# NILOIDE/A.I.gar

Measured on AMD Instinct MI355X. Metric: env-steps/sec at 4096 bots x 100k pellets; 1/2/4/8 MI355X scaling, higher is better.
Workload: dtype f64; 1 GPU; C3: 4096 bots, 100000 pellets, 1152 viruses, split p=0.0025, eject p=0.01, field 4800, obs 854 floats/bot; start: data/c3_t50.npz (tick 50, mean cell mass 17.45, max 51.3) + 30 untimed random-policy ticks to settle; policy=random, parallelism=single-gpu

## Files before the change

aigar_amd/csrc/aigar_dev.h:

```cpp
#pragma once
#include <stdint.h>

#include "../../include/aigar.h"

namespace aigar {

#ifdef AIGAR_FLOOR
#ifdef AIGAR_FLOOR_OPAQUE
#define FLOOR(k) \
  if ((((AIGAR_FLOOR) >> (k)) & 1) && d.A > 0) return
#else
#define FLOOR(k) \
  if (((AIGAR_FLOOR) >> (k)) & 1) return
#endif
#else
#define FLOOR(k)
#endif

struct ArenaCtl {
  int64_t seq_next;
  int64_t tick;
  int64_t tick_sp;
  uint64_t key0, key1, ctr_pellet, ctr_virus;
  int64_t seq_base_upd;
// ... 91 lines not shown
  int tile_flags;
  int tile_nx, tile_ny;
  int tile_gate;
  int hcap, hrec, nh;
  int *t_holder;
  int *t_obsby;
  int *t_holive;
  uint8_t *t_hodefer;
  int *t_hoslot;
  int own_bx0, own_bx1, own_by0, own_by1;
  int loc_bx0, loc_bx1, loc_by0, loc_by1;
  TileRec *outbox;
  const TileRec *inbox;
  int *ticket;
  int *kill_list;
  double *spec_x, *spec_y, *spec_m;
  double pow_n032[17];
  int cshift;
  int cshift_c;
  int Pcap, Ecap, Vcap, Wcap, EVcap;
  int PR;
  int PS;
  int PD;
  int PH1;
  int virus_enabled;
  double max_pellets, max_viruses;
  int G, L;
  uint32_t obs_ch, obs_ex;
  int flags;
  int pp_par;
  ArenaCtl *ctl;
  int *p_alive, *p_respawn, *p_ncells, *p_split, *p_eject, *p_pend;
  double *p_cmdx, *p_cmdy;
  double *p_fx, *p_fy, *p_fs, *p_mass;
  int *p_split_lh;
  uint8_t *p_role;
  int *p_time;
  double *o_last_mass;
  uint8_t *p_list;
  int *p_newc, *p_newb, *p_seqoff, *p_bloboff;
  int *p_heavy;
  double *c_x, *c_y, *c_m, *c_r, *c_vx, *c_vy, *c_svx, *c_svy, *c_mt;
  int *c_svc;
  uint32_t *c_flags;
  int64_t *c_seq;
  uint8_t *c_active;
  double *sp_r, *sp_svx, *sp_svy;
  double *sb_x, *sb_y, *sb_svx, *sb_svy;
  uint8_t *sb_slot;
  PelRec *pel;
  int *pel_col;
  PelRec *pn;
  int *pn_col;
  uint8_t *pel_dead;
  int *pel_rank;
  int *pstart;
  int *pncnt;
  uint64_t *pel_owner;
  double *b_x, *b_y, *b_m, *b_r, *b_vx, *b_vy, *b_svx, *b_svy;
  int *b_svc;
  int64_t *b_seq, *b_ej;
  int *b_col;
  uint32_t *b_flags;
  uint64_t *b_owner;
  int *bstart, *bitems, *b_rank;
  uint64_t *bmap;
  double *v_x, *v_y, *v_m, *v_r, *v_vx, *v_vy, *v_svx, *v_svy;
  int *v_svc;
  int64_t *v_seq;
  uint32_t *v_flags;
  int *v_active;
  int *vcnt, *vstart, *vitems, *v_rank;
  int *ccnt, *cstart, *citems, *c_rank;
  int *cgcnt;
  unsigned long long *occ;
  int *occ_cnt;
  int occ_words;
  int *dead;
  int *work, *work2;
  int *f_list;
  uint8_t *f_cnt;
  uint8_t *f_done;
  int *resp_slot;
  int64_t *ev;
  double *o_lastfov;
  double *o_self_lf, *o_self_slf, *o_en_lf, *o_en_slf;
  double *o_act_cur, *o_act_prev;
  unsigned long long *scan_state;
  unsigned long long *pl_state;
  int pl_tiles;
  int scan_tiles;
  int OBcap;
  unsigned long long *ob_used;
  uint32_t *ob_epoch;
  int64_t *ob_seq;
  double *ob_m, *ob_r;
  uint32_t *ob_mask;
  uint8_t *ob_own;
  int *ob_perm;
  uint64_t *ob_wmask;
  double *sc;
  ScoreCtl *sc_ctl;
};
enum { SC_N = 0, SC_SUM = 1, SC_MAX = 2, SC_DEAD = 3 };

constexpr int FCAP = 32;

struct RandomPolicy {
  int on;
  double ps, pe;
  uint64_t salt;
};

}
```

aigar_amd/csrc/api.hip:

```cpp
#include <dlfcn.h>
#include <hip/hip_runtime.h>

#include <algorithm>
#include <cmath>
#include <cstdarg>
#include <cstdio>
#include <cstdlib>
#include <cstring>
#include <string>
#include <type_traits>
#include <vector>

#include "../../include/aigar.h"
#include "aigar_dev.h"
#include "aigar_sem.h"

namespace aigar {
void launch_tick(const Dev &d, hipStream_t s, int rounds, int64_t *scr_k, int *scr_v,
                 const RandomPolicy *rp = nullptr);
void launch_tick_pre(const Dev &d, hipStream_t s, int64_t *scr_k, int *scr_v, const RandomPolicy *rp);
void launch_tick_post(const Dev &d, hipStream_t s, int64_t *scr_k, int *scr_v);
void launch_tile_pass(const Dev &d, hipStream_t s, int rounds, int64_t *scr_k, int *scr_v, int first);
void launch_tile_policy(const Dev &d, hipStream_t s, int greedy_split, uint8_t *mask, int cap);
void launch_tile_cmd_apply(const Dev &d, hipStream_t s, int box_recs);
// ... 441 lines not shown
    d.own_bx1 = (ix + 1) * d.cols / tx;
    d.own_by0 = iy * d.cols / ty;
    d.own_by1 = (iy + 1) * d.cols / ty;
    d.loc_bx0 = std::max(0, d.own_bx0 - hb);
    d.loc_bx1 = std::min(d.cols, d.own_bx1 + hb);
    d.loc_by0 = std::max(0, d.own_by0 - hb);
    d.loc_by1 = std::min(d.cols, d.own_by1 + hb);
  }
  d.tile_nx = tx;
  d.tile_ny = ty;
  d.tile_gate = 0;
  d.tcap = cfg->tile_cap > 0 ? cfg->tile_cap : 2048;
  d.bm_words = (int)(((size_t)kMaxCells * d.NP + 255) / 256 * 4);
  {
    const uint32_t ch = cfg->obs_channels;
    d.nh = ((ch & (AIGAR_OBS_SELF_LF | AIGAR_OBS_SELF_SLF)) ? 1 : 0) + ((ch & AIGAR_OBS_SELF_SLF) ? 1 : 0) +
           ((ch & (AIGAR_OBS_ENEMY_LF | AIGAR_OBS_ENEMY_SLF)) ? 1 : 0) + ((ch & AIGAR_OBS_ENEMY_SLF) ? 1 : 0);
    d.hrec = 1 + (d.nh * G * G + 3) / 4;
    d.hcap = std::min(kHcapMax, std::max(16, d.tcap / 64));
  }
  h->box_recs = 1 + d.tcap + std::max(d.bm_words / 4, d.hcap * d.hrec);
  for (int k = 0; k <= kMaxCells; k++) d.pow_n032[k] = aigar_math::pow_glibc((double)k, 0.32);
  d.cshift = 3;
  while ((((d.cols + (1 << d.cshift) - 1) >> d.cshift) * ((d.cols + (1 << d.cshift) - 1) >> d.cshift)) > 4096)
    d.cshift++;
  d.cshift_c = 0;
  while ((((d.cols + (1 << d.cshift_c) - 1) >> d.cshift_c) * ((d.cols + (1 << d.cshift_c) - 1) >> d.cshift_c)) > 4096)
    d.cshift_c++;
  if (hipStreamCreateWithFlags(&h->stream, hipStreamNonBlocking) != hipSuccess) {
    delete h;
    return fail("hipStreamCreate failed");
  }
  const size_t A = d.A, NP = d.NP, C = (size_t)kMaxCells * NP, H1 = (size_t)d.H + 1, GG = (size_t)G * G;
  bool ok = true;
#define AL(field, T, n)                     \
  do {                                      \
    d.field = dalloc<T>(h, (n));            \
    ok = ok && d.field != nullptr;          \
  } while (0)
#ifndef AIGAR_NO_ARENA
  for (int pass = 0; pass < 2; pass++) {
    h->arena_sizing = pass == 0;
    if (pass == 1) {
      h->arena_size = h->arena_used;
      h->arena_used = 0;
      void *base = nullptr;
      if (hipMalloc(&base, h->arena_size) != hipSuccess) {
        ok = false;
        break;
      }
      h->allocs.push_back(base);
      (void)hipMemset(base, 0, h->arena_size);
      h->arena = (char *)base;
    }
#endif
  AL(ctl, ArenaCtl, A);
  AL(p_alive, int, NP); AL(p_respawn, int, NP); AL(p_ncells, int, NP); AL(p_split, int, NP); AL(p_eject, int, NP);
  AL(p_pend, int, NP); AL(p_cmdx, double, NP); AL(p_cmdy, double, NP); AL(p_list, uint8_t, C);
  AL(p_newc, int, NP); AL(p_heavy, int, NP); AL(p_newb, int, NP); AL(p_seqoff, int, NP); AL(p_bloboff, int, NP);
  AL(c_x, double, C); AL(c_y, double, C); AL(c_m, double, C); AL(c_r, double, C); AL(c_vx, double, C);
  AL(c_vy, double, C); AL(c_svx, double, C); AL(c_svy, double, C); AL(c_mt, double, C); AL(c_svc, int, C);
  AL(c_flags, uint32_t, C); AL(c_seq, int64_t, C); AL(c_active, uint8_t, C);
  AL(sp_r, double, C); AL(sp_svx, double, C); AL(sp_svy, double, C);
  AL(sb_x, double, C); AL(sb_y, double, C); AL(sb_svx, double, C); AL(sb_svy, double, C); AL(sb_slot, uint8_t, C);
  const size_t P = A * d.Pcap, PSA = A * d.PS, PDA = A * d.PD, PHA = A * d.PH1;
  AL(pel, PelRec, PSA); AL(pel_col, int, PSA);
  AL(pn, PelRec, P); AL(pn_col, int, P);
  AL(pel_dead, uint8_t, PDA); AL(pel_rank, int, P); AL(pncnt, int, PHA); AL(pstart, int, PHA);
  AL(pel_owner, uint64_t, PDA);
  const size_t E = A * d.Ecap, V = A * d.Vcap;
  AL(b_x, double, E); AL(b_y, double, E); AL(b_m, double, E); AL(b_r, double, E); AL(b_vx, double, E);
  AL(b_vy, double, E); AL(b_svx, double, E); AL(b_svy, double, E); AL(b_svc, int, E); AL(b_seq, int64_t, E);
  AL(b_ej, int64_t, E); AL(b_flags, uint32_t, E); AL(b_owner, uint64_t, E); AL(b_col, int, E);
  AL(bstart, int, A * H1); AL(bitems, int, E); AL(b_rank, int, E); AL(bmap, uint64_t, A * 64);
  AL(v_x, double, V); AL(v_y, double, V); AL(v_m, double, V); AL(v_r, double, V); AL(v_vx, double, V);
  AL(v_vy, double, V); AL(v_svx, double, V); AL(v_svy, double, V); AL(v_svc, int, V); AL(v_seq, int64_t, V);
  AL(v_flags, uint32_t, V); AL(v_active, int, V);
  AL(vcnt, int, A * H1); AL(vstart, int, A * H1); AL(vitems, int, V); AL(v_rank, int, V);
  AL(ccnt, int, A * H1); AL(cstart, int, A * H1); AL(citems, int, C); AL(c_rank, int, C);
  AL(cgcnt, int, A * 2 * 4100);
  AL(occ, unsigned long long, A * d.occ_words); AL(occ_cnt, int, A * d.H);
  AL(dead, int, NP); AL(work, int, A * d.Wcap); AL(work2, int, A * d.Wcap);
  AL(f_list, int, C * FCAP); AL(f_cnt, uint8_t, C); AL(f_done, uint8_t, C);
  AL(resp_slot, int, NP);
  AL(ev, int64_t, A * d.EVcap * 5);
  AL(o_lastfov, double, NP); AL(o_self_lf, double, NP * GG); AL(o_self_slf, double, NP * GG);
  AL(o_en_lf, double, NP * GG); AL(o_en_slf, double, NP * GG); AL(o_act_cur, double, NP * 4);
  AL(o_act_prev, double, NP * 4);
  d.OBcap = (int)std::min<size_t>(std::max<size_t>(1u << 20, 64 * NP), (size_t)1 << 24);
  AL(scan_state, unsigned long long, 2 * A * d.scan_tiles);
  AL(pl_state, unsigned long long, A * d.pl_tiles);
  AL(ticket, int, 16);
  AL(kill_list, int, P); AL(spec_x, double, A * 64); AL(spec_y, double, A * 64); AL(spec_m, double, A * 64); 
  AL(ob_used, unsigned long long, 1);
  AL(ob_epoch, uint32_t, 1);
  AL(p_split_lh, int, NP);
  AL(p_role, uint8_t, NP);
  AL(p_time, int, NP);
  AL(o_last_mass, double, NP);
  if (d.tiled) {
    AL(t_holder, int, NP);
    AL(t_obsby, int, NP);
    AL(t_holive, int, NP);
    AL(t_hodefer, uint8_t, NP);
    AL(t_hoslot, int, d.hcap);
    AL(outbox, TileRec, h->box_recs);
    TileRec *ib = nullptr;
    ib = dalloc<TileRec>(h, (size_t)h->box_recs * d.ntiles);
    ok = ok && ib != nullptr;
    d.inbox = ib;
  }
  AL(p_fx, double, NP); AL(p_fy, double, NP); AL(p_fs, double, NP); AL(p_mass, double, NP); AL(ob_seq, int64_t, d.OBcap); AL(ob_m, double, d.OBcap); AL(ob_r, double, d.OBcap);
  AL(ob_mask, uint32_t, d.OBcap); AL(ob_own, uint8_t, d.OBcap); AL(ob_perm, int, d.OBcap);
  d.ob_wmask = nullptr;
  if (G > 16) AL(ob_wmask, uint64_t, 4 * (size_t)d.OBcap);
  d.sc = nullptr;
  d.sc_ctl = nullptr;
  if (cfg->flags & AIGAR_FLAG_SCORE) {
    AL(sc, double, 4 * NP);
    AL(sc_ctl, ScoreCtl, 1);
  }
#undef AL
  h->scr_k = dalloc<int64_t>(h, A * d.Wcap);
  h->scr_v = dalloc<int>(h, A * d.Wcap);
  h->d_cmd = dalloc<double>(h, NP * 4);
  h->d_mask = dalloc<uint8_t>(h, NP);
  h->d_nnmask = dalloc<uint8_t>(h, NP);
  h->d_stats = dalloc<double>(h, NP * 5);
  h->d_obs = dalloc<double>(h, NP * (size_t)d.L);
  h->d_rlist = dalloc<int>(h, A);
  h->d_rseed = dalloc<uint64_t>(h, A);
  if (d.sc) {
    h->d_score = dalloc<double>(h, NP * 4);
    ok = ok && h->d_score;
  }
  ok = ok && h->scr_k && h->scr_v && h->d_cmd && h->d_stats && h->d_obs && h->d_mask && h->d_nnmask && h->d_rlist &&
       h->d_rseed;
#ifndef AIGAR_NO_ARENA
  }
  h->arena_sizing = false;
  h->arena = nullptr;
#endif
  if (ok) (void)hipMemset(h->d_nnmask, 1, NP);
  if (ok && !d.tiled) {
    ok = hipHostMalloc((void **)&h->h_reset, aigar_handle::kResetSlots * A * 2 * sizeof(uint64_t),
                       hipHostMallocDefault) == hipSuccess;
    for (hipEvent_t &e : h->ev_reset) ok = ok && hipEventCreateWithFlags(&e, hipEventDisableTiming) == hipSuccess;
  }
  (void)hipEventCreate(&h->ev0);
  (void)hipEventCreate(&h->ev1);
  if (!ok) {
    free_all(h);
    delete h;
    return fail("aigar_create: device allocation failed");
  }
  if (hipDeviceSynchronize() != hipSuccess) {
    free_all(h);
    delete h;
    return fail("aigar_create: device synchronize failed");
  }
  *out = h;
  return 0;
}

extern "C" int aigar_destroy(aigar_handle *h) {
  if (!h) return 0;
  (void)hipSetDevice(h->cfg.device);
// ... 3367 lines not shown
```

aigar_amd/csrc/tick.hip:

```cpp
#include <hip/hip_runtime.h>

#include "aigar_dev.h"
#include "aigar_sem.h"
#include "aigar_wave.h"

namespace aigar {

#define GTID ((int)(blockIdx.x * blockDim.x + threadIdx.x))
#define TILE_GATE(d)                                          \
  do {                                                        \
    if ((d).tile_gate && (d).ctl[0].n_undone_glob == 0) return; \
  } while (0)

#ifdef AIGAR_PHASE_TIMING
constexpr int kPtWaves = 8192;
__device__ unsigned int g_ptw[9][kPtWaves][8];
__device__ unsigned int g_ptid[9][kPtWaves][2];
__device__ __forceinline__ void pt_ids(unsigned *o) {
  unsigned a, b;
  asm volatile("s_getreg_b32 %0, hwreg(HW_REG_HW_ID)" : "=s"(a));
  asm volatile("s_getreg_b32 %0, hwreg(HW_REG_XCC_ID)" : "=s"(b));
  o[0] = a;
  o[1] = b;
}
// ... 3717 lines not shown
        }
        nt += __popcll(bal);
      }
      if (nt > PPT_CAP) {
        if (lane == 0) set_err(d, a, ERR_CAND_CAP);
        nt = PPT_CAP;
      }
      tab.n = nt;
      wave_fence();
      pp_group_turns(d, a, mine, g_key[w], g_val[w], g_srt[w], odirty, rmax, d.dead + (size_t)a * d.B + dead0,
                     scr_k + (size_t)a * d.Wcap, &s_nd, tab);
    }
    if (lane == 0) s_rmax[w] = rmax;
  }
  __syncthreads();
  PT_SUB(5);
  PT_MARK(5, 7);
  const int nd = s_nd;
  const int64_t *dk = scr_k + (size_t)a * d.Wcap;
  int *dl = d.dead + (size_t)a * d.B + dead0;
  int rk[2], pv[2];
  for (int k = 0; k < 2; k++) {
    const int i = tid + k * T;
    rk[k] = -1;
    if (i < nd) {
      const int64_t key = dk[i];
      int r = 0;
      for (int j = 0; j < nd; j++) r += dk[j] < key;
      rk[k] = r;
      pv[k] = dl[i];
    }
  }
  if (nd > 2 * T && tid == 0) set_err(d, a, ERR_WORK_CAP);
  __syncthreads();
  for (int k = 0; k < 2; k++)
    if (rk[k] >= 0) dl[rk[k]] = pv[k];
  if (tid == 0) {
    double r = c.rmax_cell;
    for (int k = 0; k < PPG_WAVES; k++) r = fmax(r, s_rmax[k]);
    c.rmax_cell = r;
    c.n_dead = dead0 + nd;
    c.stat[6] += 1;
  }
  PT_SUB(6);
}

__device__ void spawn_pos(const Dev &d, int a, double radius, const uint64_t u[4], double &ox, double &oy) {
  const int cols = d.cols, total = d.H;
  const unsigned long long *occ = d.occ + (size_t)a * d.occ_words;
  int sb = (int)mulhi(u[0], (uint64_t)total);
  int found = -1;
  for (int pass = 0; pass < 2 && found < 0; pass++) {
    int lo = pass == 0 ? sb : 0, hi = pass == 0 ? total : sb;
    for (int b = lo; b < hi && found < 0;) {
      int wd = b >> 6;
      unsigned long long free_bits = ~occ[wd];
      free_bits &= (~0ull) << (b & 63);
      int wend = (wd + 1) << 6;
      if (wend > hi) free_bits &= (hi - (wd << 6)) >= 64 ? ~0ull : ((1ull << (hi - (wd << 6))) - 1);
      if (free_bits) found = (wd << 6) + __ffsll((long long)free_bits) - 1;
      b = wend;
    }
  }
  int64_t xp, yp;
  if (found < 0) {
    xp = ph_randint(u[1], 0, d.size);
    yp = ph_randint(u[2], 0, d.size);
  } else {
    int64_t x = found % cols;
    double y = (double)(found - x) / cols;
    int64_t left = (x - 1) * kBucket;
    double top = y * kBucket;
    xp = ph_randint(u[1], left + radius, (double)(left + kBucket) - radius);
    yp = ph_randint(u[2], top + radius, top + kBucket - radius);
  }
  ox = (double)xp;
  oy = (double)yp;
}

struct SpawnIn {
  int n_pel, n_pel_eaten, n_pnew, n_pel_glob, n_eaten_glob, n_vir;
  int64_t seq_next, tick, stat3, stat5;
  uint64_t ctr_pellet, ctr_virus;
  int n_spawn_p;
};
__device__ __forceinline__ SpawnIn spawn_in(const ArenaCtl &c) {
  return SpawnIn{c.n_pel,    c.n_pel_eaten, c.n_pnew,    c.n_pel_glob, c.n_eaten_glob, c.n_vir,
                 c.seq_next, c.tick,        c.stat[3],   c.stat[5],    c.ctr_pellet,   c.ctr_virus, 0};
}
__device__ __forceinline__ SpawnIn spawn_in_pel(const ArenaCtl &c) {
  SpawnIn in{};
  in.n_pel = c.n_pel;
  in.n_pel_eaten = c.n_pel_eaten;
  in.n_pnew = c.n_pnew;
  in.n_pel_glob = c.n_pel_glob;
  in.n_eaten_glob = c.n_eaten_glob;
  in.seq_next = c.seq_next;
  in.stat3 = c.stat[3];
  in.stat5 = c.stat[5];
  in.ctr_pellet = c.ctr_pellet;
  return in;
}
__device__ __forceinline__ SpawnIn spawn_in_rest(const ArenaCtl &c) {
  SpawnIn in{};
  in.n_vir = c.n_vir;
  in.seq_next = c.seq_next;
  in.tick = c.tick;
  in.ctr_virus = c.ctr_virus;
  in.n_spawn_p = c.n_spawn_p;
  return in;
}
__device__ __forceinline__ int spawn_counts_pel(const Dev &d, int a, int init, const SpawnIn &in);
__device__ __forceinline__ int spawn_counts_rest(const Dev &d, int a, int init, int n_resp, int n_wait, const SpawnIn &in,
                                                  int kp);
__device__ __forceinline__ void spawn_counts(const Dev &d, int a, int init, int n_resp, int n_wait, const SpawnIn &in);
__device__ void spawn_pellet_at(const Dev &d, int a, int j, double *px, double *py);
__device__ __forceinline__ void pellet_close_words(ArenaCtl &c, int nconv, int nsp) {
  c.pu_nconv = nconv;
  c.pu_nsp = nsp;
  c.pu_spec = nsp <= kSpawnAhead ? 1 : 0;
  c.n_pnew = 0;
  c.n_pel_eaten = 0;
}
__device__ __forceinline__ void pellet_close_prep(const Dev &d, int a) {
  ArenaCtl &c = d.ctl[a];
  const int nconv = c.n_pnew, nsp = c.n_spawn_p;
  const bool spec = nsp <= kSpawnAhead;
  if (!spec)
    for (int j = threadIdx.x; j < nsp; j += blockDim.x) spawn_pellet_at(d, a, j, nullptr, nullptr);
  __syncthreads();
  if (threadIdx.x == 0) pellet_close_words(c, nconv, nsp);
}
__global__ void __launch_bounds__(256) k_pp_active(Dev d, int close) {
  FLOOR(6);
  PT_BEGIN(3);
  const int nblocks = close ? (d.NP + 3) / 4 : (int)gridDim.x;
  if ((int)blockIdx.x >= nblocks + d.A) {
    const int gp = (blockIdx.x - nblocks - d.A) * 256 + threadIdx.x;
    if (gp < d.NP && d.p_alive[gp]) fov_store(d, gp, player_fov(d, gp));
    PT_MARK(3, 4);
    return;
  }
  if ((int)blockIdx.x >= nblocks) {
    const int a = blockIdx.x - nblocks;
    if (threadIdx.x == 0) (void)spawn_counts_pel(d, a, 0, spawn_in_pel(d.ctl[a]));
    __syncthreads();
    pellet_close_prep(d, a);
    PT_MARK(3, 5);
    return;
  }
  pp_active_own(d, nblocks PT_ARGS);
}
constexpr int PU_T = 256;
struct PelRowLds;
__device__ __forceinline__ void pel_row_update(const Dev &d, int a, int r, PelRowLds &L PT_PARAMS);
__device__ __forceinline__ void spawn_virus(const Dev &d, int gi);
__device__ __forceinline__ void spawn_player(const Dev &d, int gp, int j, int init, double *ox = nullptr,
                                             double *oy = nullptr);
__global__ void __launch_bounds__(1024) k_spawn_plan(Dev d, int init, int64_t *scr_k, int *scr_v, int pp,
                                                     int close) {
  FLOOR(7);
  if (close == 2 && (int)blockIdx.x >= d.A) {
    if (threadIdx.x >= PU_T) return;
    extern __shared__ __align__(16) unsigned char row_lds[];
    PT_BEGIN(8);
    const int rb = blockIdx.x - d.A, ra = rb / d.cols;
    pel_row_update(d, ra, rb - ra * d.cols, *reinterpret_cast<PelRowLds *>(row_lds) PT_ARGS);
    PT_MARK(8, 3);
    return;
  }
  __shared__ int sflag[1024];
  __shared__ int gcnt[SG_CAP + 1];
  PT_BEGIN(5);
  int a = blockIdx.x;
  if (pp) {
    extern __shared__ uint32_t pend[];
    __shared__ uint32_t s_odirty[OCC_DW];
    const bool defer = d.occ_words <= OCC_DW * 32;
    for (int i = threadIdx.x; i < OCC_DW; i += blockDim.x) s_odirty[i] = 0;
    for (int i = threadIdx.x; i < FOVM_BITS / 32; i += blockDim.x) fov_marks()[i] = 0;
    __syncthreads();
    pp_pass(d, a, scr_k, scr_v, pend, defer ? s_odirty : nullptr PT_ARGS);
    __syncthreads();
    if (defer) occ_rebuild_dirty(d, a, s_odirty);
    __syncthreads();
    PT_SUB(7);
  }
  PT_MARK(5, 1);
  ArenaCtl &c = d.ctl[a];
  const int T = blockDim.x, tid = threadIdx.x;
  const uint32_t dirty = c.dirty;
  for (int kind = 0; kind < 2; kind++) {
    if (!(dirty & (kind == 0 ? DIRTY_VIRUS : DIRTY_BLOB))) continue;
    if (kind == 1 && c.n_blob < 2 * c.n_blob_live + 256 && c.n_blob < d.Ecap / 2) {
      const int cc = cgrid_cols(d);
      const int ncell = d.cstart[(size_t)a * (d.H + 1) + cc * cc];
      if (c.n_blob + min(2 * ncell, kMaxCells * d.B) <= d.Ecap) continue;
    }
    int n = kind == 0 ? c.n_vir : c.n_blob;
    int cap = kind == 0 ? d.Vcap : d.Ecap;
    int out = 0;
    for (int base = 0; base < n; base += T) {
      int i = base + tid;
      size_t g = (size_t)a * cap + i;
      bool alive = i < n && ((kind == 0 ? d.v_flags[g] : d.b_flags[g]) & F_ALIVE);
      double f0 = 0, f1 = 0, f2 = 0, f3 = 0, f4 = 0, f5 = 0, f6 = 0, f7 = 0;
      int svc = 0, col = -1;
      int64_t s = 0, e = 0;
      uint32_t fl = 0;
      if (alive) {
        if (kind == 0) {
          f0 = d.v_x[g]; f1 = d.v_y[g]; f2 = d.v_m[g]; f3 = d.v_r[g]; f4 = d.v_vx[g]; f5 = d.v_vy[g];
          f6 = d.v_svx[g]; f7 = d.v_svy[g]; svc = d.v_svc[g]; s = d.v_seq[g]; fl = d.v_flags[g];
        } else {
          f0 = d.b_x[g]; f1 = d.b_y[g]; f2 = d.b_m[g]; f3 = d.b_r[g]; f4 = d.b_vx[g]; f5 = d.b_vy[g];
          f6 = d.b_svx[g]; f7 = d.b_svy[g]; svc = d.b_svc[g]; s = d.b_seq[g]; e = d.b_ej[g]; fl = d.b_flags[g];
          col = d.b_col[g];
        }
      }
      int chunk;
      const int pos = out + block_rank(alive, sflag, &chunk);
      if (alive) {
        size_t o = (size_t)a * cap + pos;
        if (kind == 0) {
          d.v_x[o] = f0; d.v_y[o] = f1; d.v_m[o] = f2; d.v_r[o] = f3; d.v_vx[o] = f4; d.v_vy[o] = f5;
          d.v_svx[o] = f6; d.v_svy[o] = f7; d.v_svc[o] = svc; d.v_seq[o] = s; d.v_flags[o] = fl;
        } else {
          d.b_x[o] = f0; d.b_y[o] = f1; d.b_m[o] = f2; d.b_r[o] = f3; d.b_vx[o] = f4; d.b_vy[o] = f5;
          d.b_svx[o] = f6; d.b_svy[o] = f7; d.b_svc[o] = svc; d.b_seq[o] = s; d.b_ej[o] = e; d.b_flags[o] = fl;
          d.b_col[o] = col;
        }
      }
      out += chunk;
      __syncthreads();
    }
    for (int i = out + tid; i < n; i += T) {
      size_t g = (size_t)a * cap + i;
      if (kind == 0) d.v_flags[g] = 0;
      else d.b_flags[g] = 0;
    }
    __syncthreads();
    if (tid == 0) {
      if (kind == 0) c.n_vir = out;
      else c.n_blob = out;
    }
    __syncthreads();
  }
  PT_MARK(5, 2);
  if (d.virus_enabled && (dirty & DIRTY_VIRUS)) grid_small_build<2>(d, a, gcnt, sflag);
  PT_MARK(5, 3);
  int n_resp = 0, n_wait = 0;
  SpawnIn sin{};
  if (tid == 0) sin = close == 2 ? spawn_in_rest(c) : spawn_in(c);
  uint32_t ob_ep = 0;
  if (tid == 0 && close == 2 && a == 0) ob_ep = *d.ob_epoch;
  if (!init) {
    const int nd = c.n_dead;
    int *dl = d.dead + (size_t)a * d.B, *rl = d.resp_slot + (size_t)a * d.B;
    for (int base = 0; base < nd; base += T) {
      const int i = base + tid;
      int p = -1;
      bool rsp = false;
      if (i < nd) {
        p = dl[i];
        rsp = d.p_respawn[(size_t)a * d.B + p] == 0;
      }
      int tr, tw;
      const int rr = block_rank(i < nd && rsp, sflag, &tr);
      const int rw = block_rank(i < nd && !rsp, sflag, &tw);
      if (i < nd) rl[p] = rsp ? n_resp + rr : -1;
      if (i < nd && !rsp) dl[n_wait + rw] = p;
      if (close == 2 && i < nd && rsp) fov_mark(p);
      n_resp += tr;
      n_wait += tw;
    }
  }
  __shared__ int s_kv;
  if (tid == 0) {
    if (close == 2) {
      s_kv = spawn_counts_rest(d, a, init, n_resp, n_wait, sin, sin.n_spawn_p);
      c.tick = sin.tick + 1;
      if (a == 0) *d.ob_epoch = 0x80000000u | ((ob_ep + 1) & 0x7FFFFFFFu);
    } else {
      spawn_counts(d, a, init, n_resp, n_wait, sin);
    }
  }
  __syncthreads();
  PT_MARK(5, 4);
  if (close == 1) {
    __syncthreads();
    pellet_close_prep(d, a);
  }
  if (close == 2) {
    for (int j = tid; j < s_kv; j += T) spawn_virus(d, a * d.Vcap + j);
    for (int p = tid; p < d.B; p += T) {
      if (!fov_marked(p)) continue;
      const int gp = a * d.B + p;
      const bool alive = d.p_alive[gp];
      const int j = d.resp_slot[gp];
      Fov f;
      if (alive) {
        f = player_fov(d, gp);
      } else {
        if (j < 0) continue;
        double x, y;
        spawn_player(d, gp, j, 0, &x, &y);
        f = player_fov_of(d, 1, [&](int, double &cx, double &cy, double &cm, double &cr) {
          cx = x;
          cy = y;
          cm = kStartMass;
          cr = radius_of(kStartMass);
        });
      }
      fov_store(d, gp, f);
      if (f.rmax > 0) atomic_max_pos(&c.rmax_cell, f.rmax);
    }
  }
  PT_MARK(5, 5);
}

__device__ __forceinline__ void spawn_counts(const Dev &d, int a, int init, int n_resp, int n_wait, const SpawnIn &in) {
  const int kp = spawn_counts_pel(d, a, init, in);
  (void)spawn_counts_rest(d, a, init, n_resp, n_wait, in, kp);
}
__device__ __forceinline__ int spawn_counts_pel(const Dev &d, int a, int init, const SpawnIn &in) {
  ArenaCtl &c = d.ctl[a];
  const int n_pel = in.n_pel, n_pel_eaten = in.n_pel_eaten, n_pnew = in.n_pnew;
  const int n_pel_glob = in.n_pel_glob, n_eaten_glob = in.n_eaten_glob;
  const int64_t seq_next = in.seq_next, stat3 = in.stat3, stat5 = in.stat5;
  const uint64_t ctr_pellet = in.ctr_pellet;
  uint32_t err = 0;
  const int alive_p = d.tiled ? n_pel_glob - n_eaten_glob + n_pnew : n_pel - n_pel_eaten + n_pnew;
  int kp = 0;
  if ((double)alive_p < d.max_pellets) kp = (int)ceil(d.max_pellets) - alive_p;
  if (alive_p + kp > d.Pcap || n_pnew + kp > d.Pcap) {
    err |= ERR_PELLET_CAP;
    kp = max(0, min(d.Pcap - alive_p, d.Pcap - n_pnew));
  }
  if (err) set_err(d, a, err);
  c.seq_base_spawn = seq_next;
  c.ctr_pellet_base = ctr_pellet;
  c.ctr_pellet = ctr_pellet + kp;
  c.n_spawn_p = kp;
  c.n_pel_glob = alive_p + kp;
  if (!init) {
    c.stat[3] = stat3 + (d.tiled ? n_eaten_glob : n_pel_eaten);
    c.stat[5] = stat5 + kp;
  }
  return kp;
}
__device__ __forceinline__ int spawn_counts_rest(const Dev &d, int a, int init, int n_resp, int n_wait, const SpawnIn &in,
                                                  int kp) {
  ArenaCtl &c = d.ctl[a];
  const int n_vir = in.n_vir;
  const int64_t seq_next = in.seq_next, tick = in.tick;
  const uint64_t ctr_virus = in.ctr_virus;
  uint32_t err = 0;
  int kv = 0;
  if (d.virus_enabled && (double)n_vir < d.max_viruses) kv = (int)ceil(d.max_viruses) - n_vir;
  if (n_vir + kv > d.Vcap) {
    err |= ERR_VIRUS_CAP;
    kv = d.Vcap - n_vir;
  }
  const int np = init ? d.B : n_resp;
  c.dirty = 0;
  if (err) set_err(d, a, err);
  c.ctr_virus_base = ctr_virus;
  c.ctr_virus = ctr_virus + kv;
  c.vir_base_spawn = n_vir;
  c.n_spawn_v = kv;
  c.n_vir = n_vir + kv;
  if (!init) {
    c.n_dead = n_wait;
    c.tick_sp = tick;
  }
  c.n_spawn_pl = np;
  c.seq_next = seq_next + kp + kv + (init ? 0 : np);
  return kv;
}

__global__ void k_pnew_commit(Dev d) {
  int a = GTID;
  if (a >= d.A) return;
  d.ctl[a].n_pnew += d.ctl[a].n_spawn_p;
}

__device__ __forceinline__ void spawn_pellet_rec(const Dev &d, const ArenaCtl &c, int j, double &x, double &y,
                                                 double &m, int64_t &seq) {
  uint64_t u[4];
  philox(c.ctr_pellet_base + j, ST_PELLET, 0, 0, c.key0, c.key1, u);
  x = (double)(int64_t)mulhi(u[0], (uint64_t)d.size);
  y = (double)(int64_t)mulhi(u[1], (uint64_t)d.size);
  const int64_t sr = (int64_t)mulhi(u[2], 50);
  m = (sr > 50 - 4) ? (double)(50 - sr) : 1.0;
  seq = c.seq_base_spawn + j;
}
__device__ void spawn_pellet_at(const Dev &d, int a, int j, double *px, double *py) {
  const ArenaCtl &c = d.ctl[a];
  double x, y, m;
// ... 928 lines not shown
```

Before: 50.14 million env-steps/s.

## Move list compaction and dead-player partition into earlier pp_active arena blocks

Moves virus and blob list compaction, the virus grid rebuild and the dead-player respawn partition out of the close==2 pass and into the extra per-arena blocks of k_pp_active, which now run a shared lists_plan helper. A new resp_list array records the respawning players, so the final pass iterates only over those and over fov-marked alive players through a bitmask scan instead of all B players. The final pass also drops the 1024-int shared scratch array. This shortens the serial tail of the tick, at the cost of more work in the earlier kernel and a reordering that has to keep the spawn counts and the dirty state consistent.

```diff
diff --git a/aigar_amd/csrc/aigar_dev.h b/aigar_amd/csrc/aigar_dev.h
--- a/aigar_amd/csrc/aigar_dev.h
+++ b/aigar_amd/csrc/aigar_dev.h
@@ -197,6 +197,7 @@
   uint8_t *f_cnt;
   uint8_t *f_done;
   int *resp_slot;
+  int *resp_list;
   int64_t *ev;
   double *o_lastfov;
   double *o_self_lf, *o_self_slf, *o_en_lf, *o_en_slf;
diff --git a/aigar_amd/csrc/api.hip b/aigar_amd/csrc/api.hip
--- a/aigar_amd/csrc/api.hip
+++ b/aigar_amd/csrc/api.hip
@@ -547,7 +547,7 @@
   AL(occ, unsigned long long, A * d.occ_words); AL(occ_cnt, int, A * d.H);
   AL(dead, int, NP); AL(work, int, A * d.Wcap); AL(work2, int, A * d.Wcap);
   AL(f_list, int, C * FCAP); AL(f_cnt, uint8_t, C); AL(f_done, uint8_t, C);
-  AL(resp_slot, int, NP);
+  AL(resp_slot, int, NP); AL(resp_list, int, NP);
   AL(ev, int64_t, A * d.EVcap * 5);
   AL(o_lastfov, double, NP); AL(o_self_lf, double, NP * GG); AL(o_self_slf, double, NP * GG);
   AL(o_en_lf, double, NP * GG); AL(o_en_slf, double, NP * GG); AL(o_act_cur, double, NP * 4);
diff --git a/aigar_amd/csrc/tick.hip b/aigar_amd/csrc/tick.hip
--- a/aigar_amd/csrc/tick.hip
+++ b/aigar_amd/csrc/tick.hip
@@ -3823,33 +3823,10 @@
   int n_pel, n_pel_eaten, n_pnew, n_pel_glob, n_eaten_glob, n_vir;
   int64_t seq_next, tick, stat3, stat5;
   uint64_t ctr_pellet, ctr_virus;
-  int n_spawn_p;
 };
 __device__ __forceinline__ SpawnIn spawn_in(const ArenaCtl &c) {
   return SpawnIn{c.n_pel,    c.n_pel_eaten, c.n_pnew,    c.n_pel_glob, c.n_eaten_glob, c.n_vir,
-                 c.seq_next, c.tick,        c.stat[3],   c.stat[5],    c.ctr_pellet,   c.ctr_virus, 0};
-}
-__device__ __forceinline__ SpawnIn spawn_in_pel(const ArenaCtl &c) {
-  SpawnIn in{};
-  in.n_pel = c.n_pel;
-  in.n_pel_eaten = c.n_pel_eaten;
-  in.n_pnew = c.n_pnew;
-  in.n_pel_glob = c.n_pel_glob;
-  in.n_eaten_glob = c.n_eaten_glob;
-  in.seq_next = c.seq_next;
-  in.stat3 = c.stat[3];
-  in.stat5 = c.stat[5];
-  in.ctr_pellet = c.ctr_pellet;
-  return in;
-}
-__device__ __forceinline__ SpawnIn spawn_in_rest(const ArenaCtl &c) {
-  SpawnIn in{};
-  in.n_vir = c.n_vir;
-  in.seq_next = c.seq_next;
-  in.tick = c.tick;
-  in.ctr_virus = c.ctr_virus;
-  in.n_spawn_p = c.n_spawn_p;
-  return in;
+                 c.seq_next, c.tick,        c.stat[3],   c.stat[5],    c.ctr_pellet,   c.ctr_virus};
 }
 __device__ __forceinline__ int spawn_counts_pel(const Dev &d, int a, int init, const SpawnIn &in);
 __device__ __forceinline__ int spawn_counts_rest(const Dev &d, int a, int init, int n_resp, int n_wait, const SpawnIn &in,
@@ -3872,6 +3849,110 @@
   __syncthreads();
   if (threadIdx.x == 0) pellet_close_words(c, nconv, nsp);
 }
+template <int KIND>
+__device__ __forceinline__ int list_compact(const Dev &d, int a, int n, int *sh) {
+  const int T = blockDim.x, tid = threadIdx.x;
+  const int cap = KIND == 0 ? d.Vcap : d.Ecap;
+  int out = 0;
+  for (int base = 0; base < n; base += T) {
+    int i = base + tid;
+    size_t g = (size_t)a * cap + i;
+    bool alive = i < n && ((KIND == 0 ? d.v_flags[g] : d.b_flags[g]) & F_ALIVE);
+    double f0 = 0, f1 = 0, f2 = 0, f3 = 0, f4 = 0, f5 = 0, f6 = 0, f7 = 0;
+    int svc = 0, col = -1;
+    int64_t s = 0, e = 0;
+    uint32_t fl = 0;
+    if (alive) {
+      if (KIND == 0) {
+        f0 = d.v_x[g]; f1 = d.v_y[g]; f2 = d.v_m[g]; f3 = d.v_r[g]; f4 = d.v_vx[g]; f5 = d.v_vy[g];
+        f6 = d.v_svx[g]; f7 = d.v_svy[g]; svc = d.v_svc[g]; s = d.v_seq[g]; fl = d.v_flags[g];
+      } else {
+        f0 = d.b_x[g]; f1 = d.b_y[g]; f2 = d.b_m[g]; f3 = d.b_r[g]; f4 = d.b_vx[g]; f5 = d.b_vy[g];
+        f6 = d.b_svx[g]; f7 = d.b_svy[g]; svc = d.b_svc[g]; s = d.b_seq[g]; e = d.b_ej[g]; fl = d.b_flags[g];
+        col = d.b_col[g];
+      }
+    }
+    int chunk;
+    const int pos = out + block_rank(alive, sh, &chunk);
+    if (alive) {
+      size_t o = (size_t)a * cap + pos;
+      if (KIND == 0) {
+        d.v_x[o] = f0; d.v_y[o] = f1; d.v_m[o] = f2; d.v_r[o] = f3; d.v_vx[o] = f4; d.v_vy[o] = f5;
+        d.v_svx[o] = f6; d.v_svy[o] = f7; d.v_svc[o] = svc; d.v_seq[o] = s; d.v_flags[o] = fl;
+      } else {
+        d.b_x[o] = f0; d.b_y[o] = f1; d.b_m[o] = f2; d.b_r[o] = f3; d.b_vx[o] = f4; d.b_vy[o] = f5;
+        d.b_svx[o] = f6; d.b_svy[o] = f7; d.b_svc[o] = svc; d.b_seq[o] = s; d.b_ej[o] = e; d.b_flags[o] = fl;
+        d.b_col[o] = col;
+      }
+    }
+    out += chunk;
+    __syncthreads();
+  }
+  for (int i = out + tid; i < n; i += T) {
+    size_t g = (size_t)a * cap + i;
+    if (KIND == 0) d.v_flags[g] = 0;
+    else d.b_flags[g] = 0;
+  }
+  __syncthreads();
+  if (tid == 0) {
+    if (KIND == 0) d.ctl[a].n_vir = out;
+    else d.ctl[a].n_blob = out;
+  }
+  __syncthreads();
+  return out;
+}
+__device__ __forceinline__ bool blob_compact_due(const Dev &d, int n_blob, int n_blob_live, int ncell) {
+  if (n_blob < 2 * n_blob_live + 256 && n_blob < d.Ecap / 2) return n_blob + min(2 * ncell, kMaxCells * d.B) > d.Ecap;
+  return true;
+}
+__device__ __forceinline__ void dead_partition(const Dev &d, int a, int nd, int p_first, int *sh, int &n_resp,
+                                               int &n_wait) {
+  const int T = blockDim.x, tid = threadIdx.x;
+  int *dl = d.dead + (size_t)a * d.B, *rs = d.resp_slot + (size_t)a * d.B, *rl = d.resp_list + (size_t)a * d.B;
+  n_resp = n_wait = 0;
+  for (int base = 0; base < nd; base += T) {
+    const int i = base + tid;
+    const bool in = i < nd;
+    const int p = base == 0 ? p_first : in ? dl[i] : 0;
+    const bool rsp = in && d.p_respawn[(size_t)a * d.B + p] == 0;
+    int tr, tw;
+    const int rr = block_rank(rsp, sh, &tr);
+    const int rw = block_rank(in && !rsp, sh, &tw);
+    if (in) rs[p] = rsp ? n_resp + rr : -1;
+    if (rsp) rl[n_resp + rr] = p;
+    if (in && !rsp) dl[n_wait + rw] = p;
+    n_resp += tr;
+    n_wait += tw;
+  }
+}
+template <int PTK>
+__device__ __forceinline__ void lists_plan(const Dev &d, int a, int init, int *sh, int *gcnt PT_PARAMS) {
+  ArenaCtl &c = d.ctl[a];
+  const int tid = threadIdx.x;
+  const int p_first = !init && tid < d.B ? d.dead[(size_t)a * d.B + tid] : 0;
+  const uint32_t dirty = c.dirty;
+  int n_vir = c.n_vir;
+  const int n_blob = c.n_blob, n_blob_live = c.n_blob_live, nd = c.n_dead;
+  const int cc = cgrid_cols(d);
+  const int ncell = d.cstart[(size_t)a * (d.H + 1) + cc * cc];
+  SpawnIn sin{};
+  if (tid == 0) sin = spawn_in(c);
+  if (dirty & DIRTY_VIRUS) n_vir = list_compact<0>(d, a, n_vir, sh);
+  if ((dirty & DIRTY_BLOB) && blob_compact_due(d, n_blob, n_blob_live, ncell)) (void)list_compact<1>(d, a, n_blob, sh);
+  if (PTK == 5) PT_MARK(5, 2);
+  if (d.virus_enabled && (dirty & DIRTY_VIRUS)) grid_small_build<2>(d, a, gcnt, sh);
+  if (PTK == 5) PT_MARK(5, 3);
+  if (PTK == 3) PT_MARK(3, 6);
+  int n_resp = 0, n_wait = 0;
+  if (!init) dead_partition(d, a, nd, p_first, sh, n_resp, n_wait);
+  if (PTK == 3) PT_MARK(3, 7);
+  if (tid == 0) {
+    sin.n_vir = n_vir;
+    spawn_counts(d, a, init, n_resp, n_wait, sin);
+  }
+  __syncthreads();
+  if (PTK == 5) PT_MARK(5, 4);
+}
 __global__ void __launch_bounds__(256) k_pp_active(Dev d, int close) {
   FLOOR(6);
   PT_BEGIN(3);
@@ -3883,9 +3964,9 @@
     return;
   }
   if ((int)blockIdx.x >= nblocks) {
+    __shared__ int l_sh[32], l_gcnt[SG_CAP + 1];
     const int a = blockIdx.x - nblocks;
-    if (threadIdx.x == 0) (void)spawn_counts_pel(d, a, 0, spawn_in_pel(d.ctl[a]));
-    __syncthreads();
+    lists_plan<3>(d, a, 0, l_sh, l_gcnt PT_ARGS);
     pellet_close_prep(d, a);
     PT_MARK(3, 5);
     return;
@@ -3910,10 +3991,18 @@
     PT_MARK(8, 3);
     return;
   }
-  __shared__ int sflag[1024];
+  __shared__ int sflag[32];
   __shared__ int gcnt[SG_CAP + 1];
   PT_BEGIN(5);
   int a = blockIdx.x;
+  ArenaCtl &c = d.ctl[a];
+  const int T = blockDim.x, tid = threadIdx.x;
+  int n_resp = 0, n_spawn_v = 0, rp_first = 0;
+  if (close == 2) {
+    n_resp = __builtin_amdgcn_readfirstlane(c.n_spawn_pl);
+    n_spawn_v = __builtin_amdgcn_readfirstlane(c.n_spawn_v);
+    if (tid < d.B) rp_first = d.resp_list[(size_t)a * d.B + tid];
+  }
   if (pp) {
     extern __shared__ uint32_t pend[];
     __shared__ uint32_t s_odirty[OCC_DW];
@@ -3928,134 +4017,52 @@
     PT_SUB(7);
   }
   PT_MARK(5, 1);
-  ArenaCtl &c = d.ctl[a];
-  const int T = blockDim.x, tid = threadIdx.x;
-  const uint32_t dirty = c.dirty;
-  for (int kind = 0; kind < 2; kind++) {
-    if (!(dirty & (kind == 0 ? DIRTY_VIRUS : DIRTY_BLOB))) continue;
-    if (kind == 1 && c.n_blob < 2 * c.n_blob_live + 256 && c.n_blob < d.Ecap / 2) {
-      const int cc = cgrid_cols(d);
-      const int ncell = d.cstart[(size_t)a * (d.H + 1) + cc * cc];
-      if (c.n_blob + min(2 * ncell, kMaxCells * d.B) <= d.Ecap) continue;
-    }
-    int n = kind == 0 ? c.n_vir : c.n_blob;
-    int cap = kind == 0 ? d.Vcap : d.Ecap;
-    int out = 0;
-    for (int base = 0; base < n; base += T) {
-      int i = base + tid;
-      size_t g = (size_t)a * cap + i;
-      bool alive = i < n && ((kind == 0 ? d.v_flags[g] : d.b_flags[g]) & F_ALIVE);
-      double f0 = 0, f1 = 0, f2 = 0, f3 = 0, f4 = 0, f5 = 0, f6 = 0, f7 = 0;
-      int svc = 0, col = -1;
-      int64_t s = 0, e = 0;
-      uint32_t fl = 0;
-      if (alive) {
-        if (kind == 0) {
-          f0 = d.v_x[g]; f1 = d.v_y[g]; f2 = d.v_m[g]; f3 = d.v_r[g]; f4 = d.v_vx[g]; f5 = d.v_vy[g];
-          f6 = d.v_svx[g]; f7 = d.v_svy[g]; svc = d.v_svc[g]; s = d.v_seq[g]; fl = d.v_flags[g];
-        } else {
-          f0 = d.b_x[g]; f1 = d.b_y[g]; f2 = d.b_m[g]; f3 = d.b_r[g]; f4 = d.b_vx[g]; f5 = d.b_vy[g];
-          f6 = d.b_svx[g]; f7 = d.b_svy[g]; svc = d.b_svc[g]; s = d.b_seq[g]; e = d.b_ej[g]; fl = d.b_flags[g];
-          col = d.b_col[g];
-        }
-      }
-      int chunk;
-      const int pos = out + block_rank(alive, sflag, &chunk);
-      if (alive) {
-        size_t o = (size_t)a * cap + pos;
-        if (kind == 0) {
-          d.v_x[o] = f0; d.v_y[o] = f1; d.v_m[o] = f2; d.v_r[o] = f3; d.v_vx[o] = f4; d.v_vy[o] = f5;
-          d.v_svx[o] = f6; d.v_svy[o] = f7; d.v_svc[o] = svc; d.v_seq[o] = s; d.v_flags[o] = fl;
-        } else {
-          d.b_x[o] = f0; d.b_y[o] = f1; d.b_m[o] = f2; d.b_r[o] = f3; d.b_vx[o] = f4; d.b_vy[o] = f5;
-          d.b_svx[o] = f6; d.b_svy[o] = f7; d.b_svc[o] = svc; d.b_seq[o] = s; d.b_ej[o] = e; d.b_flags[o] = fl;
-          d.b_col[o] = col;
-        }
-      }
-      out += chunk;
-      __syncthreads();
-    }
-    for (int i = out + tid; i < n; i += T) {
-      size_t g = (size_t)a * cap + i;
-      if (kind == 0) d.v_flags[g] = 0;
-      else d.b_flags[g] = 0;
-    }
-    __syncthreads();
-    if (tid == 0) {
-      if (kind == 0) c.n_vir = out;
-      else c.n_blob = out;
-    }
-    __syncthreads();
-  }
-  PT_MARK(5, 2);
-  if (d.virus_enabled && (dirty & DIRTY_VIRUS)) grid_small_build<2>(d, a, gcnt, sflag);
-  PT_MARK(5, 3);
-  int n_resp = 0, n_wait = 0;
-  SpawnIn sin{};
-  if (tid == 0) sin = close == 2 ? spawn_in_rest(c) : spawn_in(c);
-  uint32_t ob_ep = 0;
-  if (tid == 0 && close == 2 && a == 0) ob_ep = *d.ob_epoch;
-  if (!init) {
-    const int nd = c.n_dead;
-    int *dl = d.dead + (size_t)a * d.B, *rl = d.resp_slot + (size_t)a * d.B;
-    for (int base = 0; base < nd; base += T) {
-      const int i = base + tid;
-      int p = -1;
-      bool rsp = false;
-      if (i < nd) {
-        p = dl[i];
-        rsp = d.p_respawn[(size_t)a * d.B + p] == 0;
-      }
-      int tr, tw;
-      const int rr = block_rank(i < nd && rsp, sflag, &tr);
-      const int rw = block_rank(i < nd && !rsp, sflag, &tw);
-      if (i < nd) rl[p] = rsp ? n_resp + rr : -1;
-      if (i < nd && !rsp) dl[n_wait + rw] = p;
-      if (close == 2 && i < nd && rsp) fov_mark(p);
-      n_resp += tr;
-      n_wait += tw;
-    }
-  }
-  __shared__ int s_kv;
-  if (tid == 0) {
-    if (close == 2) {
-      s_kv = spawn_counts_rest(d, a, init, n_resp, n_wait, sin, sin.n_spawn_p);
-      c.tick = sin.tick + 1;
-      if (a == 0) *d.ob_epoch = 0x80000000u | ((ob_ep + 1) & 0x7FFFFFFFu);
-    } else {
-      spawn_counts(d, a, init, n_resp, n_wait, sin);
+  if (close != 2) {
+    lists_plan<5>(d, a, init, sflag, gcnt PT_ARGS);
+    if (close == 1) pellet_close_prep(d, a);
+    PT_MARK(5, 5);
+    return;
+  }
+  for (int j = tid; j < n_spawn_v; j += T) spawn_virus(d, a * d.Vcap + j);
+  for (int s = tid; s < FOVM_BITS / 8; s += T) {
+    uint32_t m = (fov_marks()[s >> 2] >> ((s & 3) * 8)) & 0xFFu;
+    while (m) {
+      const int b = __ffs(m) - 1;
+      m &= m - 1;
+      for (int p = s * 8 + b; p < d.B; p += FOVM_BITS) {
+        const int gp = a * d.B + p;
+        if (!d.p_alive[gp]) continue;
+        const Fov f = player_fov(d, gp);
+        fov_store(d, gp, f);
+        if (f.rmax > 0) atomic_max_pos(&c.rmax_cell, f.rmax);
+      }
     }
   }
   __syncthreads();
   PT_MARK(5, 4);
-  if (close == 1) {
-    __syncthreads();
-    pellet_close_prep(d, a);
-  }
-  if (close == 2) {
-    for (int j = tid; j < s_kv; j += T) spawn_virus(d, a * d.Vcap + j);
-    for (int p = tid; p < d.B; p += T) {
-      if (!fov_marked(p)) continue;
-      const int gp = a * d.B + p;
-      const bool alive = d.p_alive[gp];
-      const int j = d.resp_slot[gp];
-      Fov f;
-      if (alive) {
-        f = player_fov(d, gp);
-      } else {
-        if (j < 0) continue;
-        double x, y;
-        spawn_player(d, gp, j, 0, &x, &y);
-        f = player_fov_of(d, 1, [&](int, double &cx, double &cy, double &cm, double &cr) {
-          cx = x;
-          cy = y;
-          cm = kStartMass;
-          cr = radius_of(kStartMass);
-        });
-      }
-      fov_store(d, gp, f);
-      if (f.rmax > 0) atomic_max_pos(&c.rmax_cell, f.rmax);
-    }
+  int64_t tick = 0;
+  uint32_t ob_ep = 0;
+  if (tid == 0) {
+    tick = c.tick;
+    if (a == 0) ob_ep = *d.ob_epoch;
+  }
+  if (tid == 0) {
+    c.tick = tick + 1;
+    if (a == 0) *d.ob_epoch = 0x80000000u | ((ob_ep + 1) & 0x7FFFFFFFu);
+  }
+  for (int j = tid; j < n_resp; j += T) {
+    const int p = j == tid ? rp_first : d.resp_list[(size_t)a * d.B + j];
+    const int gp = a * d.B + p;
+    double x, y;
+    spawn_player(d, gp, j, 0, &x, &y);
+    const Fov f = player_fov_of(d, 1, [&](int, double &cx, double &cy, double &cm, double &cr) {
+      cx = x;
+      cy = y;
+      cm = kStartMass;
+      cr = radius_of(kStartMass);
+    });
+    fov_store(d, gp, f);
+    if (f.rmax > 0) atomic_max_pos(&c.rmax_cell, f.rmax);
   }
   PT_MARK(5, 5);
 }
```

Result: faster. 50.96 million env-steps/s (median of 6 runs) (+1.6%).
